# arkworks-rs/gemini

Measured on AMD Instinct MI355X. Metric: BLS12-381 G1 MSM throughput, higher is better.
Workload: dtype u32x12 Montgomery Fq (381-bit integer), u32x8 Fr; 1 GPU; 2^20 G1 MSM per GPU (BASELINE configs[1]: 2^20 G1 MSM on one MI355X); pairs_per_gpu=1048576

## Files before the change

gemini_amd/csrc/capi.hip:

```cpp
#include <cstring>
#include <vector>

#include "ctx.hpp"
#include "host_field.hpp"

namespace gm {

static thread_local char g_err[512] = "";
void set_error(const char* fmt, ...) {
  va_list ap;
  va_start(ap, fmt);
  vsnprintf(g_err, sizeof g_err, fmt, ap);
  va_end(ap);
}
int hip_fail(hipError_t e, const char* what, const char* file, int line) {
  set_error("HIP error %d (%s) in %s at %s:%d", (int)e, hipGetErrorString(e), what, file, line);
  return e == hipErrorOutOfMemory ? GM_ENOMEM : GM_EHIP;
}

MemStats& mem_stats() {
  static MemStats* m = new MemStats;
  return *m;
}
void MemStats::note_cached(ptrdiff_t delta) {
// ... 309 lines not shown
  if (const char* e = getenv("GM_POOL_MAX_GB")) C->pool.max_pooled = (size_t)strtoull(e, nullptr, 10) << 30;
  int prio_lo = 0, prio_hi = 0;
  GM_HIP(hipDeviceGetStreamPriorityRange(&prio_lo, &prio_hi));
  const bool prio = getenv("GM_STREAM_PRIO") && atoi(getenv("GM_STREAM_PRIO")) != 0;
  GM_HIP(hipStreamCreateWithPriority(&C->stream, hipStreamNonBlocking, prio ? prio_lo : 0));
  for (int k = 0; k < MSM_SMALL_LANES; k++) GM_HIP(hipStreamCreateWithPriority(&C->small_stream[k], hipStreamNonBlocking, prio ? prio_hi : 0));
  GM_HIP(hipStreamCreateWithPriority(&C->stream_b, hipStreamNonBlocking, prio ? prio_hi : 0));
  {
    const char* e = getenv("GM_CU_SPLIT");
    const int ncu = C->cu_count, per_xcd = ncu / 8;
    int T = e ? atoi(e) : (ncu == 256 ? per_xcd : 0);
    static const bool raw_env = getenv("GM_CU_SPLIT_RAW") != nullptr;
    if (!raw_env && per_xcd > 0) T = T / per_xcd * per_xcd;
    if (ncu % 8 == 0 && T > 0 && T < ncu) {
      const int words = (ncu + 31) / 32, xcds = T / per_xcd, stride = ncu / T;
      std::vector<uint32_t> m_tail((size_t)words, 0u), m_acc((size_t)words, 0u);
      int taken = 0;
      for (int i = 0; i < ncu; i++) {
        const bool tail = raw_env ? (taken < T && i % stride == 0) : (i % 8 < xcds);
        (tail ? m_tail : m_acc)[(size_t)i >> 5] |= 1u << (i & 31);
        taken += tail ? 1 : 0;
      }
      bool ok = true;
      for (int k = 0; k < 2 + MSM_SMALL_LANES && ok; k++) {
        ok = hipExtStreamCreateWithCUMask(&C->part_acc[k], (uint32_t)words, m_acc.data()) == hipSuccess &&
             hipExtStreamCreateWithCUMask(&C->part_tail[k], (uint32_t)words, m_tail.data()) == hipSuccess;
      }
      if (ok) {
        C->cu_split = T;
        static bool registered = false;
        if (!registered) {
          registered = true;
          atexit([] {
            Context* c = g_ctx;
            if (!c || !c->cu_split) return;
            c->cu_split = 0;
            for (int k = 0; k < 2 + MSM_SMALL_LANES; k++) {
              if (c->part_acc[k]) (void)hipStreamSynchronize(c->part_acc[k]), (void)hipStreamDestroy(c->part_acc[k]);
              if (c->part_tail[k]) (void)hipStreamSynchronize(c->part_tail[k]), (void)hipStreamDestroy(c->part_tail[k]);
              c->part_acc[k] = c->part_tail[k] = nullptr;
            }
          });
        }
      } else {
        (void)hipGetLastError();
      }
    }
  }
  GM_HIP(hipHostMalloc((void**)&C->host_small, 1 << 16, hipHostMallocDefault));
  GM_HIP(hipHostMalloc((void**)&C->sc_desc_host, SC_DESC_SLOTS * SC_DESC_SLOT, hipHostMallocDefault));
  GM_HIP(gm::raw_malloc(&C->sc_desc_dev, SC_DESC_SLOTS * SC_DESC_SLOT));
  for (auto& e : C->sc_desc_copied) GM_HIP(hipEventCreateWithFlags(&e, hipEventDisableTiming));
  if (const char* e = getenv("GM_ZERO_COPY")) C->zero_copy = atoi(e);
  g_ctx = C;
  return GM_OK;
}

void gm_shutdown(void) {
  std::lock_guard<std::mutex> lk(g_ctx_mu);
  if (!g_ctx) return;
  Context* C = g_ctx;
  (void)hipStreamSynchronize(C->stream);
  for (auto& kv : C->bases) {
    bases_free_tables(kv.second.get());
    if (kv.second->phi) (void)gm::raw_free(kv.second->phi);
    if (kv.second->d) (void)gm::raw_free(kv.second->d);
  }
  for (auto& kv : C->vecs)
    if (kv.second->d) (void)gm::raw_free(kv.second->d);
  for (auto& kv : C->msm_streams) msm_stream_destroy(C, kv.second.get());
  C->pool.release_all();
  for (auto& kv : C->provers) sc_destroy(kv.second.get());
  for (auto& kv : C->space_provers) sp_destroy(C, kv.second.get());
  for (auto& kv : C->herring_g1) hg1_destroy(C, kv.second.get());
  C->partial_bufs.release_all();
  for (auto& kv : C->indices)
    if (kv.second->d) (void)gm::raw_free(kv.second->d);
  for (auto& kv : C->matrices) {
    if (kv.second->rowptr) (void)gm::raw_free(kv.second->rowptr);
    if (kv.second->cols) (void)gm::raw_free(kv.second->cols);
    if (kv.second->vals) (void)gm::raw_free(kv.second->vals);
  }
  auto release_ws = [](MsmWorkspace& w) {
    for (DevBuf* b : {&w.scalars, &w.counts, &w.offsets, &w.cursor, &w.entries, &w.tmp_entries, &w.sortmeta, &w.buckets, &w.pk[0], &w.pk[1], &w.pp[0],
                      &w.pp[1], &w.rows, &w.cols, &w.planes, &w.misc, &w.lvl_cnt, &w.lvl_pos, &w.lvl_pts[0], &w.lvl_pts[1], &w.lvl_keys[0],
                      &w.lvl_keys[1], &w.lvl_prefix, &w.lvl_lane, &w.lvl_entries, &w.lvl_n})
      b->release();
    for (int k = 0; k < MSM_SLOTS; k++)
      if (w.host_planes[k]) (void)hipHostFree(w.host_planes[k]);
    if (w.have_done_ev) {
      for (int e = 0; e < MSM_SLOTS; e++) (void)hipEventDestroy(w.done_ev[e]);
    }
  };
  release_ws(C->msm);
  release_ws(C->msm_b);
  if (C->stream_b) (void)hipStreamDestroy(C->stream_b);
  for (int k = 0; k < MSM_SMALL_LANES; k++) {
    release_ws(C->msm_small[k]);
    if (C->small_stream[k]) (void)hipStreamDestroy(C->small_stream[k]);
  }
  for (int k = 0; k < 2 + MSM_SMALL_LANES; k++) {
    if (C->part_acc[k]) (void)hipStreamDestroy(C->part_acc[k]);
    if (C->part_tail[k]) (void)hipStreamDestroy(C->part_tail[k]);
  }
  C->cu_split = 0;
  if (C->host_small) (void)hipHostFree(C->host_small);
  if (C->sc_desc_host) (void)hipHostFree(C->sc_desc_host);
  if (C->sc_desc_dev) (void)gm::raw_free(C->sc_desc_dev);
  for (auto& e : C->sc_desc_copied)
    if (e) (void)hipEventDestroy(e);
  if (C->host_batch) (void)hipHostFree(C->host_batch);
  (void)hipStreamDestroy(C->stream);
  delete C;
  g_ctx = nullptr;
}

int gm_prof_enable(int on) {
  GM_CTX();
  C->prof.on = on != 0;
  C->prof.only_stage = on == 2 ? (int)PROF_ACC0 : -1;
  for (int s = 0; s < PROF_NSTAGES; s++) {
    C->prof.ms[s] = 0;
    C->prof.count[s] = 0;
    C->prof.pending[0][s] = C->prof.pending[1][s] = false;
  }
  C->prof.acc0_cycles = C->prof.acc0_ticks = 0;
  return GM_OK;
}
int gm_prof_read_clock(double* acc0_mhz) {
  GM_CTX();
  GM_CHECK(acc0_mhz != nullptr, GM_EINVAL, "prof_read_clock: null pointer");
  *acc0_mhz = C->prof.acc0_ticks > 0 ? C->prof.acc0_cycles / C->prof.acc0_ticks * 100.0 : 0.0;
  return GM_OK;
}
int gm_prof_read(double* ms_out, uint64_t* count_out, int n) {
  GM_CTX();
  GM_CHECK(n >= 0 && n <= PROF_NSTAGES, GM_EINVAL, "prof_read: n = %d, at most %d stages", n, (int)PROF_NSTAGES);
  for (int s = 0; s < n; s++) {
    if (ms_out) ms_out[s] = C->prof.ms[s];
    if (count_out) count_out[s] = C->prof.count[s];
  }
  return GM_OK;
}

int gm_set_msm_table_min(size_t n) {
  GM_CTX();
  C->msm_table_min = n;
  return GM_OK;
}

int gm_set_auto_tables(int on, size_t max_bytes) {
  GM_CTX();
  C->auto_tables = on != 0;
  C->auto_tables_max = max_bytes;
  return GM_OK;
}

int gm_pool_trim(void) {
  GM_CTX();
  C->pool.release_all();
  return GM_OK;
}

int gm_mem_stats(uint64_t out[12]) {
  GM_CTX();
  GM_CHECK(out != nullptr, GM_EINVAL, "gm_mem_stats: null output");
  size_t free_b = 0, total_b = 0;
// ... 1268 lines not shown
```

gemini_amd/csrc/ctx.hpp:

```cpp
#pragma once
#include <hip/hip_runtime.h>

#include <atomic>
#include <cstdarg>
#include <cstdint>
#include <cstdio>
#include <map>
#include <memory>
#include <mutex>
#include <string>
#include <unordered_map>
#include <vector>

#include "../../include/gemini_hip.h"

namespace gm {

void set_error(const char* fmt, ...);
int hip_fail(hipError_t e, const char* what, const char* file, int line);

#define GM_HIP(expr)                                                     \
  do {                                                                   \
    hipError_t _e = (expr);                                              \
    if (_e != hipSuccess) return ::gm::hip_fail(_e, #expr, __FILE__, __LINE__); \
// ... 68 lines not shown
  size_t round = 0, tot_rounds = 0;
  uint64_t pair_offset = 0;
  bool herring = false;
  uint8_t* partials = nullptr;
  uint64_t* host_partials = nullptr;
  unsigned pending_blocks = 0;
  bool on_host = false;
  std::vector<uint64_t> hf, hg;
  uint64_t host_msg[8];
  bool host_msg_pending = false;
  std::mutex mu;
};
constexpr size_t SC_HOST_TAIL = 256;
constexpr size_t SC_DESC_SLOT = (size_t)32 << 10;
constexpr unsigned SC_DESC_SLOTS = 8;

struct SpaceProver {
  uint8_t* f = nullptr;
  uint8_t* g = nullptr;
  size_t nf = 0, ng = 0, fcap = 0, gcap = 0;
  bool borrowed = false;
  std::vector<uint64_t> challenges, twisted;
  uint64_t twist[4];
  size_t round = 0, tot_rounds = 0;
  uint8_t* tables = nullptr;
  size_t tables_cap = 0;
  uint8_t *wf_lo = nullptr, *wf_hi = nullptr, *wg_lo = nullptr, *wg_hi = nullptr;
  uint8_t* partials = nullptr;
  uint64_t* host_partials = nullptr;
  std::mutex mu;
};

struct HerringG1 {
  uint8_t* f[2] = {nullptr, nullptr};
  uint8_t* g[2] = {nullptr, nullptr};
  size_t fcap[2] = {0, 0}, gcap[2] = {0, 0};
  int cur = 0;
  size_t nf = 0, ng = 0;
  uint64_t twist[4];
  size_t round = 0, tot_rounds = 0;
  uint8_t* tmp = nullptr;
  size_t tmpcap = 0;
  std::mutex mu;
};

struct MsmWorkspace;
struct MsmPending {
  MsmWorkspace* ws = nullptr;
  int slot = 0;
  bool empty = true;
  int Wb = 0, c = 0, m = 0;
  uint32_t nbits = 0, wf[3] = {0, 0, 0};
  size_t plane_off[3] = {0, 0, 0};
  size_t plane_count = 0;
  int multi_levels = 0;
  int multi_W = 0;
};
struct MsmStreamSlot {
  uint8_t *raw = nullptr, *packed = nullptr, *scalars = nullptr;
  size_t raw_cap = 0, packed_cap = 0, scalars_cap = 0;
  hipEvent_t copied;
  bool have_ev = false;
  bool inflight = false;
  MsmPending P;
};
struct MsmStream {
  std::mutex mu;
  size_t chunk = 0, stride = 96;
  int mont = 0;
  uint64_t bases_handle = 0;
  int64_t base0 = 0, next_base = 0, step = 1;
  MsmStreamSlot s[2];
  int cur = 0;
  size_t fill = 0, total = 0;
  hipStream_t copy = nullptr;
  uint64_t acc[18];
  bool acc_set = false;
};

constexpr int MSM_SLOTS = 4;
constexpr int MSM_SMALL_LANES = 6;
struct MsmWorkspace {
  DevBuf scalars, counts, offsets, cursor, entries, tmp_entries, sortmeta, buckets, pk[2], pp[2], rows, cols, planes, misc;
  DevBuf clk;
  DevBuf lvl_cnt, lvl_pos, lvl_pts[2], lvl_keys[2], lvl_prefix, lvl_lane, lvl_entries, lvl_n;
  uint64_t* host_planes[MSM_SLOTS] = {};
  size_t host_planes_cap[MSM_SLOTS] = {};
  hipEvent_t done_ev[MSM_SLOTS];
  hipEvent_t sort_ev, acc_ev;
  bool have_done_ev = false;
};

enum ProfStage { PROF_DIGITS = 0, PROF_SCAN, PROF_SCATTER, PROF_ACC0, PROF_MERGE, PROF_REDUCE, PROF_SC_ROUND, PROF_EXTFREQ, PROF_NSTAGES };
struct Profiler {
  bool on = false;
  int only_stage = -1;
  hipEvent_t ev[2][2 * PROF_NSTAGES];
  bool have_events = false;
  bool pending[2][PROF_NSTAGES] = {};
  double ms[PROF_NSTAGES] = {};
  uint64_t count[PROF_NSTAGES] = {};
  double acc0_cycles = 0, acc0_ticks = 0;
  void begin(int part, int stage, hipStream_t st);
  void end(int part, int stage, hipStream_t st);
  void begin(int stage, hipStream_t st) { begin(0, stage, st); }
  void end(int stage, hipStream_t st) { end(0, stage, st); }
  void collect();
};

struct DevPool {
  std::mutex mu;
  std::multimap<size_t, void*> free_list;
  size_t pooled_bytes = 0;
  size_t max_pooled = (size_t)96 << 30;
  int alloc(size_t bytes, void** p, size_t* cap);
  void free(void* p, size_t cap);
  void release_all();
};

struct PartialBufs {
  std::mutex mu;
  std::vector<std::pair<uint8_t*, uint64_t*>> free_pairs;
  int take(uint8_t** dev, uint64_t** host);
  void give(uint8_t* dev, uint64_t* host);
  void release_all();
};
constexpr size_t PARTIAL_BUF_BYTES = 512 * 2 * 32;

struct Context {
  int device = -1;
  PartialBufs partial_bufs;
  DevPool pool;
  Profiler prof;
  hipStream_t stream = nullptr;
  std::mutex mu;
  std::recursive_mutex msm_mu;
  std::recursive_mutex fr_mu;
  uint64_t next_handle = 1;
  std::unordered_map<uint64_t, std::unique_ptr<Bases>> bases;
  std::unordered_map<uint64_t, std::unique_ptr<FrVec>> vecs;
  std::unordered_map<uint64_t, std::unique_ptr<Sumcheck>> provers;
  std::unordered_map<uint64_t, std::unique_ptr<SparseMatrix>> matrices;
  std::unordered_map<uint64_t, std::unique_ptr<SpaceProver>> space_provers;
  std::unordered_map<uint64_t, std::unique_ptr<HerringG1>> herring_g1;
  std::unordered_map<uint64_t, std::unique_ptr<MsmStream>> msm_streams;
  std::unordered_map<uint64_t, std::unique_ptr<IdxVec>> indices;
  MsmWorkspace msm;
  MsmWorkspace msm_small[MSM_SMALL_LANES];
  hipStream_t small_stream[MSM_SMALL_LANES] = {};
  MsmWorkspace msm_b;
  hipStream_t stream_b = nullptr;
  int cu_split = 0;
  hipStream_t part_acc[2 + MSM_SMALL_LANES] = {};
  hipStream_t part_tail[2 + MSM_SMALL_LANES] = {};
  hipEvent_t start_ev;
  bool have_start_ev = false;
  DevBuf fr_scratch;
  uint64_t* host_small = nullptr;
  uint8_t* sc_desc_host = nullptr;
  uint8_t* sc_desc_dev = nullptr;
  hipEvent_t sc_desc_copied[SC_DESC_SLOTS] = {};
  unsigned sc_desc_next = 0;
  uint64_t* host_batch = nullptr;
  size_t host_batch_cap = 0;
  int msm_c_override = 0;
  int msm_glv = 0;
// ... 63 lines not shown
```

gemini_amd/csrc/msm.hip:

```cpp
#include <algorithm>
#include <atomic>
#include <chrono>
#include <condition_variable>
#include <cstdlib>
#include <cstring>
#include <functional>
#include <sched.h>
#include <cstdio>
#include <thread>
#include <vector>

#include "ctx.hpp"
#include "g1.cuh"
#include "host_field.hpp"

namespace gm {

constexpr uint32_t KEY_INV = 0xffffffffu;
constexpr int XYZZ_BYTES = 192;
constexpr int AFF_BYTES = 96;

struct DigitIter {
  uint32_t s[8];
  uint32_t carry;
// ... 830 lines not shown
      if (tab_stride) {
        const uint32_t lo = (uint32_t)e & 0x7fffffffu;
        idx = (long long)(lo >> ENTRY_W_SHIFT) * tab_stride + first + step * (long long)(lo & ((1u << ENTRY_W_SHIFT) - 1u));
      } else {
        idx = first + step * (long long)(e & 0x3fffffffull);
      }
      const uint8_t* src = (phi != nullptr && ((e >> ENTRY_HALF_SHIFT) & 1ull)) ? phi : bases;
      return reinterpret_cast<const gm_u4v*>(src + (size_t)idx * AFF_BYTES);
    };
    uint64_t e = entry_at(start);
    const gm_u4v* bp = base_of(e);
    gm_u4v x0 = bp[0], x1 = bp[1], x2 = bp[2], y0 = bp[3], y1 = bp[4], y2 = bp[5];
    for (uint64_t i = start; i < end; i++) {
      uint64_t en = 0;
      gm_u4v n0 = x0, n1 = x1, n2 = x2, n3 = y0, n4 = y1, n5 = y2;
      if (i + 1 < end) {
        en = entry_at(i + 1);
        const gm_u4v* np = base_of(en);
        asm volatile(
            "global_load_dwordx4 %0, %6, off\n\t"
            "global_load_dwordx4 %1, %6, off offset:16\n\t"
            "global_load_dwordx4 %2, %6, off offset:32\n\t"
            "global_load_dwordx4 %3, %6, off offset:48\n\t"
            "global_load_dwordx4 %4, %6, off offset:64\n\t"
            "global_load_dwordx4 %5, %6, off offset:80"
            : "=&v"(n0), "=&v"(n1), "=&v"(n2), "=&v"(n3), "=&v"(n4), "=&v"(n5)
            : "v"(np));
      }
      const uint32_t key = (uint32_t)(e >> 32);
      if (key != cur) {
        if (cur != KEY_INV) {
          if (first_run) {
            head_key = cur;
            acc30_store(pp + (size_t)(2 * (size_t)t) * XYZZ30_BYTES, acc);
            first_run = false;
          } else {
            acc30_store(buckets + (size_t)cur * XYZZ30_BYTES, acc);
          }
        }
        cur = key;
        acc30_set_identity(acc);
      }
      const uint32_t nz = x0.x | x0.y | x0.z | x0.w | x1.x | x1.y | x1.z | x1.w | x2.x | x2.y | x2.z | x2.w | y0.x | y0.y | y0.z | y0.w |
                          y1.x | y1.y | y1.z | y1.w | y2.x | y2.y | y2.z | y2.w;
      if (nz != 0) {
        const uint32_t neg = (uint32_t)(e >> 31) & 1u;
        (void)g1_madd30_asm(acc, x0, x1, x2, y0, y1, y2, neg);
      }
      asm volatile("s_waitcnt vmcnt(0)" : "+v"(n0), "+v"(n1), "+v"(n2), "+v"(n3), "+v"(n4), "+v"(n5));
      e = en;
      x0 = n0; x1 = n1; x2 = n2; y0 = n3; y1 = n4; y2 = n5;
    }
    if (first_run) {
      head_key = cur;
      acc30_store(pp + (size_t)(2 * (size_t)t) * XYZZ30_BYTES, acc);
    } else {
      tail_key = cur;
      acc30_store(pp + (size_t)(2 * (size_t)t + 1) * XYZZ30_BYTES, acc);
    }
  }
  pk[2 * (size_t)t] = head_key;
  pk[2 * (size_t)t + 1] = tail_key;
  if (t == 0 && clk != nullptr) {
    clk[0] = (unsigned long long)(clock64() - clk_c0);
    clk[1] = (unsigned long long)(wall_clock64() - clk_w0);
  }
}

#ifdef GM_EXPERIMENTS
#include "msm_levels.inc"
#endif

__global__ __launch_bounds__(64) void k_merge(const uint32_t* __restrict__ keys_in, const uint8_t* __restrict__ pts_in,
                                              uint32_t E, uint32_t* __restrict__ keys_out,
                                              uint8_t* __restrict__ pts_out, uint8_t* __restrict__ buckets,
                                              int final_level) {
  __shared__ __attribute__((aligned(16))) uint8_t lds[128 * XYZZ30_BYTES];
  const int lane = threadIdx.x;
  const uint32_t wave = blockIdx.x;
  const uint32_t s0 = wave * 128u + 2u * lane;
  uint32_t hk = s0 < E ? keys_in[s0] : KEY_INV;
  uint32_t tk = s0 + 1 < E ? keys_in[s0 + 1] : KEY_INV;
  uint32_t hs = 2 * lane, ts = 2 * lane + 1;
  auto copy_rec = [](void* dst, const void* src) {
    const gm_u4v* s = reinterpret_cast<const gm_u4v*>(src);
    gm_u4v* d = reinterpret_cast<gm_u4v*>(dst);
#pragma unroll
    for (int i = 0; i < 13; i++) d[i] = s[i];
  };
  auto add_slots = [&](uint32_t dst_slot, uint32_t src_slot, Acc30& a) {
    Acc30 o;
    acc30_load(a, lds + dst_slot * XYZZ30_BYTES);
    acc30_load(o, lds + src_slot * XYZZ30_BYTES);
    acc30_add(a, o);
  };
  if (hk != KEY_INV) copy_rec(lds + hs * XYZZ30_BYTES, pts_in + (size_t)s0 * XYZZ30_BYTES);
  if (tk != KEY_INV) copy_rec(lds + ts * XYZZ30_BYTES, pts_in + ((size_t)s0 + 1) * XYZZ30_BYTES);
  if (hk == KEY_INV && tk != KEY_INV) {
    hk = tk;
    hs = ts;
    tk = KEY_INV;
  }
  __syncthreads();
  if (hk != KEY_INV && hk == tk) {
    Acc30 a;
    add_slots(hs, ts, a);
    acc30_store(lds + hs * XYZZ30_BYTES, a);
    tk = KEY_INV;
  }
  __syncthreads();

  {
    const uint32_t nhk = __shfl_down(hk, 1), nhs = __shfl_down(hs, 1), ntk = __shfl_down(tk, 1);
    const uint32_t ptk = __shfl_up(tk, 1);
    const bool give = lane < 63 && tk != KEY_INV && ntk != KEY_INV && nhk == tk;
    const bool taken = lane > 0 && tk != KEY_INV && ptk != KEY_INV && ptk == hk;
    if (__any(give)) {
      if (give) {
        Acc30 a;
        add_slots(ts, nhs, a);
        acc30_store(buckets + (size_t)tk * XYZZ30_BYTES, a);
      }
    }
    __syncthreads();
    if (taken) {
      hk = tk; hs = ts; tk = KEY_INV;
    }
    if (give) {
      if (taken) { hk = KEY_INV; } else { tk = KEY_INV; }
    }
  }

  for (int d = 1; d < 64; d <<= 1) {
    const uint32_t bhk = __shfl_down(hk, d), bhs = __shfl_down(hs, d);
    const uint32_t btk = __shfl_down(tk, d), bts = __shfl_down(ts, d);
    const bool act = (lane & (2 * d - 1)) == 0;
    bool do_add = false;
    uint32_t add_dst = 0, add_src = 0;
    uint32_t f1k = KEY_INV, f1s = 0, f2k = KEY_INV, f2s = 0;
    if (act && bhk != KEY_INV) {
      if (hk == KEY_INV) {
        hk = bhk; hs = bhs; tk = btk; ts = bts;
      } else {
        const bool a_two = tk != KEY_INV, b_two = btk != KEY_INV;
        const uint32_t alk = a_two ? tk : hk, als = a_two ? ts : hs;
        if (alk == bhk) {
          do_add = true; add_dst = als; add_src = bhs;
          if (b_two) {
            if (a_two) { f1k = alk; f1s = als; }
            tk = btk; ts = bts;
          }
        } else {
          if (a_two) { f1k = tk; f1s = ts; }
          if (b_two) { f2k = bhk; f2s = bhs; tk = btk; ts = bts; }
          else { tk = bhk; ts = bhs; }
        }
      }
    }
    if (__any(do_add)) {
      if (do_add) {
        Acc30 a;
        add_slots(add_dst, add_src, a);
        acc30_store(lds + add_dst * XYZZ30_BYTES, a);
      }
    }
    if (f1k != KEY_INV) copy_rec(buckets + (size_t)f1k * XYZZ30_BYTES, lds + f1s * XYZZ30_BYTES);
    if (f2k != KEY_INV) copy_rec(buckets + (size_t)f2k * XYZZ30_BYTES, lds + f2s * XYZZ30_BYTES);
    __syncthreads();
  }
  if (lane == 0) {
    if (final_level) {
      if (hk != KEY_INV) copy_rec(buckets + (size_t)hk * XYZZ30_BYTES, lds + hs * XYZZ30_BYTES);
      if (tk != KEY_INV) copy_rec(buckets + (size_t)tk * XYZZ30_BYTES, lds + ts * XYZZ30_BYTES);
    } else {
      keys_out[2 * (size_t)wave] = hk;
      keys_out[2 * (size_t)wave + 1] = tk;
      if (hk != KEY_INV) copy_rec(pts_out + (size_t)(2 * (size_t)wave) * XYZZ30_BYTES, lds + hs * XYZZ30_BYTES);
      if (tk != KEY_INV) copy_rec(pts_out + (size_t)(2 * (size_t)wave + 1) * XYZZ30_BYTES, lds + ts * XYZZ30_BYTES);
    }
  }
}

enum { GS_STRIDED = 0, GS_PLANE = 1 };
struct GroupSumArgs {
  const uint8_t* in;
  uint8_t* out;
  int mode;
  uint32_t n_out;
  uint32_t per_win;
  uint32_t win_stride;
  uint32_t n_lo, s_hi, s_lo, s_e, len;
  uint32_t nb;
  uint32_t lpo_shift;
  int out_canonical;
  const uint32_t* in_cnt;
};
struct GroupSumJobs {
  GroupSumArgs j[3];
  uint32_t blk_end[3];
  const uint32_t* err_src;
  uint32_t* err_dst;
  const unsigned long long* clk_src;
};

__global__ __launch_bounds__(256) void k_group_sum(GroupSumJobs J) {
  if (J.err_dst && blockIdx.x == 0 && threadIdx.x == 0) {
    *J.err_dst = *J.err_src;
    if (J.clk_src) {
      unsigned long long* d = reinterpret_cast<unsigned long long*>(J.err_dst + 2);
      d[0] = J.clk_src[0];
      d[1] = J.clk_src[1];
    }
  }
  const int job = blockIdx.x < J.blk_end[0] ? 0 : (blockIdx.x < J.blk_end[1] ? 1 : 2);
  const GroupSumArgs& a = J.j[job];
  const uint32_t blk0 = job == 0 ? 0u : J.blk_end[job - 1];
  const uint8_t* __restrict__ in = a.in;
  uint8_t* __restrict__ out = a.out;
  const uint32_t gt = (blockIdx.x - blk0) * blockDim.x + threadIdx.x;
  const uint32_t lpo = 1u << a.lpo_shift;
  const uint32_t o = gt >> a.lpo_shift, q = gt & (lpo - 1u);
  Acc30 acc;
  acc30_zero(acc);
  const uint32_t* __restrict__ in_cnt = a.in_cnt;
  auto filled = [&](size_t slot) { return in_cnt == nullptr || in_cnt[slot] != 0u; };
  auto add_rec = [&](size_t slot) {
    if (!filled(slot)) return;
    Acc30 v;
    acc30_load(v, in + slot * XYZZ30_BYTES);
    acc30_add(acc, v);
  };
  auto load_first = [&](size_t slot) {
    if (filled(slot)) acc30_load(acc, in + slot * XYZZ30_BYTES);
  };
  if (o < a.n_out) {
    const uint32_t w = o / a.per_win, r = o % a.per_win;
    const size_t base = (size_t)w * a.win_stride;
    if (a.mode == GS_STRIDED) {
      const size_t b0 = base + (size_t)(r / a.n_lo) * a.s_hi + (size_t)(r % a.n_lo) * a.s_lo;
      if (q < a.len) load_first(b0 + (size_t)q * a.s_e);
      for (uint32_t e = q + lpo; e < a.len; e += lpo) add_rec(b0 + (size_t)e * a.s_e);
    } else {
      const uint32_t nb = a.nb;
      if (r == nb) {
        const uint32_t cnt0 = nb ? (1u << (nb - 1)) : 1u;
        if (q < cnt0) load_first(base + 2u * q);
        for (uint32_t e = q + lpo; e < cnt0; e += lpo) add_rec(base + 2u * e);
      } else {
        const uint32_t half = nb ? (1u << (nb - 1)) : 0u;
        auto slot_of = [&](uint32_t e) { return ((e >> r) << (r + 1)) | (1u << r) | (e & ((1u << r) - 1u)); };
        if (q < half) load_first(base + slot_of(q));
        for (uint32_t e = q + lpo; e < half; e += lpo) add_rec(base + slot_of(e));
      }
    }
  }
#pragma unroll 1
  for (int m = (int)(lpo >> 1); m >= 1; m >>= 1) {
    Acc30 other;
    acc30_shfl_xor(other, acc, m);
    acc30_add(acc, other);
  }
  if (o < a.n_out && q == 0) {
    if (a.out_canonical) g1_store_xyzz(out + (size_t)o * XYZZ_BYTES, acc30_to_canonical(acc));
// ... 125 lines not shown
}

__global__ __launch_bounds__(256) void k_fixed_base_mul(const uint32_t* __restrict__ scalars, int mont, size_t n,
                                                        const uint8_t* __restrict__ table_aff, uint8_t* __restrict__ out_xyzz) {
  size_t i = (size_t)blockIdx.x * blockDim.x + threadIdx.x;
  if (i >= n) return;
  Fr s = fp_load<FrParams>(scalars + 8 * i);
  if (mont) s = fp_from_mont<FrParams>(s);
  G1Xyzz acc = G1Xyzz::identity();
  for (int w = 0; w < 32; w++) {
    uint32_t dgt = (s.l[w >> 2] >> (8 * (w & 3))) & 255u;
    if (dgt) {
      G1Affine p = g1_load_affine(table_aff + ((size_t)w * 256 + dgt) * AFF_BYTES);
      xyzz_madd(acc, p);
    }
  }
  g1_store_xyzz(out_xyzz + i * XYZZ_BYTES, acc);
}

__global__ __launch_bounds__(256) void k_g1_split_fold(const uint8_t* __restrict__ in, size_t n, const uint32_t* __restrict__ s8,
                                                       uint8_t* __restrict__ out) {
  const size_t m = (n + 1) / 2;
  size_t i = (size_t)blockIdx.x * blockDim.x + threadIdx.x;
  if (i >= m) return;
  G1Affine lo = g1_load_affine(in + (2 * i) * AFF_BYTES);
  G1Xyzz acc = G1Xyzz::identity();
  if (2 * i + 1 < n) {
    G1Affine hi = g1_load_affine(in + (2 * i + 1) * AFF_BYTES);
    for (int bit = 254; bit >= 0; bit--) {
      acc = xyzz_dbl(acc);
      if ((s8[bit >> 5] >> (bit & 31)) & 1u) xyzz_madd(acc, hi);
    }
  }
  xyzz_madd(acc, lo);
  G1Affine a;
  if (acc.is_identity()) {
    a.x = fqe_zero();
    a.y = fqe_zero();
  } else {
    FqE t = fq_mul(acc.zz, acc.zzz);
    FqE ti = fq_inv(t);
    a.x = fq_mul(acc.x, fq_mul(ti, acc.zzz));
    a.y = fq_mul(acc.y, fq_mul(ti, acc.zz));
  }
  g1_store_affine(out + i * AFF_BYTES, a);
}

__global__ __launch_bounds__(256) void k_table_next(const uint8_t* __restrict__ prev, uint8_t* __restrict__ next_xyzz, size_t n, int c) {
  size_t i = (size_t)blockIdx.x * blockDim.x + threadIdx.x;
  if (i >= n) return;
  G1Affine p = g1_load_affine(prev + i * AFF_BYTES);
  G1Xyzz acc = G1Xyzz::from_affine(p);
  for (int k = 0; k < c; k++) acc = xyzz_dbl(acc);
  g1_store_xyzz(next_xyzz + i * XYZZ_BYTES, acc);
}

static int ceil_log2_sz(size_t n) {
  int b = 0;
  size_t v = n > 1 ? n - 1 : 0;
  while (v) {
    b++;
    v >>= 1;
  }
  return b;
}

static int choose_window(size_t n) {
  int lg = ceil_log2_sz(n);
  static const size_t c20_min = getenv("GM_MSM_C20_MIN") ? (size_t)strtoull(getenv("GM_MSM_C20_MIN"), nullptr, 10) : ((size_t)7 << 21);
  if (n >= c20_min) return 20;
  if (lg >= 23) return 19;
  static const int c_medium = getenv("GM_MSM_C_MEDIUM") ? atoi(getenv("GM_MSM_C_MEDIUM")) : 0;
  if (c_medium && lg >= 14 && lg <= 17) return c_medium;
  if (lg >= 14) return 16;
  if (lg >= 11) return 8;
  if (lg >= 8) return lg - 4;
  if (lg >= 5) return lg + 1;
  return 4;
}

size_t msm_workspace_held(const MsmWorkspace& ws) {
  size_t b = 0;
  for (const DevBuf* d : {&ws.scalars, &ws.counts, &ws.offsets, &ws.cursor, &ws.entries, &ws.tmp_entries, &ws.sortmeta, &ws.buckets, &ws.pk[0], &ws.pk[1],
                          &ws.pp[0], &ws.pp[1], &ws.rows, &ws.cols, &ws.planes, &ws.misc, &ws.clk})
    b += d->cap;
  return b;
}
size_t msm_workspace_bound(Context* C, const Bases* bases, size_t n) {
  if (n == 0) return 0;
  n = std::min<size_t>(n, (size_t)1 << 26);
  int c = C->msm_c_override ? C->msm_c_override : choose_window(n);
  bool table = false;
  if (bases && !C->msm_c_override && n < ((size_t)1 << ENTRY_W_SHIFT)) {
    if (bases->table && n >= std::max(C->msm_table_min, bases->tab_min)) {
      c = bases->tab_c;
      table = true;
    } else {
      for (const Bases::TableSet& ts : bases->extra)
        if (n >= ts.min_n && n < ts.max_n && n <= ts.n) {
          c = ts.c;
          table = true;
          break;
        }
    }
  }
  const size_t W = (size_t)(256 + c - 1) / (size_t)c;
  const size_t N = n * W, nbuckets = (table ? 1 : W) << (c - 1);
  auto grow = [](size_t b) { return b + b / 8 + 256; };
  const size_t lanes0 = N >= ((size_t)1 << 24) ? 262144 : 131072;
  const size_t L = std::min<size_t>(256, std::max<size_t>(4, (N + lanes0 - 1) / lanes0)) + 1;
  const size_t E1 = 2 * ((N / L + 256 + 255) / 256 * 256), E2 = 2 * ((E1 + 127) / 128);
  size_t b = 2 * grow(N * 8);
  b += grow(nbuckets * XYZZ30_BYTES) + 4 * grow((nbuckets + 8192) * 4);
  b += grow(E1 * 4) + grow(E1 * XYZZ30_BYTES) + grow(E2 * 4) + grow(E2 * XYZZ30_BYTES);
  b += (size_t)W * ((size_t)3 << 14) * XYZZ30_BYTES + ((size_t)16 << 20);
  return b;
}

constexpr size_t MSM_SMALL_N = (size_t)1 << 17;
constexpr size_t MSM_SPLIT_MIN_N = (size_t)1 << 17;
static int msm_run_one(Context* C, const Bases* bases, int64_t first, int64_t step, const void* d_scalars, int mont, size_t n,
                       bool normalize, uint64_t out_jac[18]);
static int msm_run_batch_at(Context* C, const Bases* bases, int64_t first, int64_t step, const size_t* pair_offsets, const void* const* d_scalars,
                            int mont, const size_t* ns, size_t k, bool normalize, uint64_t* out_jac, const int64_t* firsts = nullptr);

struct MsmStreams {
  hipStream_t sort, acc, tail;
};
struct MsmMulti {
  bool block = false;
  int levels = 0;
  const void* scalars[MULTI_MAX_LEVELS];
  size_t n[MULTI_MAX_LEVELS];
  int64_t start[MULTI_MAX_LEVELS];
};
constexpr size_t MSM_MULTI_MAX_N = (size_t)1 << 13;
constexpr size_t MSM_MULTI_BLOCK_MAX_N = (size_t)1 << 20;
static int msm_enqueue(Context* C, MsmWorkspace& ws, MsmStreams sts, const Bases* bases, int64_t first, int64_t step, const void* d_scalars,
                       int mont, size_t n, int slot, MsmPending* P, int part = 0, int nparts = 1, const MsmMulti* multi = nullptr);
static int msm_finish_parts(Context* C, const MsmPending* parts, int nparts, bool normalize, uint64_t out_jac[18], bool use_pool = true,
                            uint64_t* const* multi_out = nullptr);
static void horner_pool_prewake();
static void horner_pool_run(int n, const std::function<void(int)>& fn);
static int msm_finish(Context* C, const MsmPending& P, bool normalize, uint64_t out_jac[18], bool use_pool = true) {
  return msm_finish_parts(C, &P, 1, normalize, out_jac, use_pool);
}

int msm_run(Context* C, const Bases* bases, int64_t first, int64_t step, const void* d_scalars, int mont, size_t n,
            bool normalize, uint64_t out_jac[18]) {
  const size_t CH = (size_t)1 << 26;
  if (n <= CH) return msm_run_one(C, bases, first, step, d_scalars, mont, n, normalize, out_jac);
  gmh::G1 acc = gmh::G1::identity();
  for (size_t off = 0; off < n; off += CH) {
    const size_t m = n - off < CH ? n - off : CH;
    uint64_t part[18];
    int rc = msm_run_one(C, bases, first + step * (int64_t)off, step, reinterpret_cast<const uint8_t*>(d_scalars) + off * 32, mont, m, false, part);
    if (rc) return rc;
    acc = acc.add(gmh::G1::from_limbs(part));
  }
  if (normalize) acc = acc.normalized();
  acc.to_limbs(out_jac);
  return GM_OK;
}

static int msm_run_one(Context* C, const Bases* bases, int64_t first, int64_t step, const void* d_scalars, int mont, size_t n,
                       bool normalize, uint64_t out_jac[18]) {
  GM_MSM_LOCK(C);
  const bool tables = bases->table != nullptr && !C->msm_c_override && n >= std::max(C->msm_table_min, bases->tab_min) &&
                      n < ((size_t)1 << ENTRY_W_SHIFT);
  const bool split = GM_GLV(1) && C->msm_split && n >= MSM_SPLIT_MIN_N && !tables && C->msm_affine_levels == 0 && C->stream_b && C->small_stream[0];
  if (!split) {
    MsmPending P;
    int rc = msm_enqueue(C, C->msm, MsmStreams{C->stream, C->stream, C->stream}, bases, first, step, d_scalars, mont, n, 0, &P);
    if (rc) return rc;
    return msm_finish(C, P, normalize, out_jac);
  }
  if (!C->have_start_ev) {
    GM_HIP(hipEventCreateWithFlags(&C->start_ev, hipEventDisableTiming));
    C->have_start_ev = true;
  }
  GM_HIP(hipEventRecord(C->start_ev, C->stream));
  GM_HIP(hipStreamWaitEvent(C->small_stream[0], C->start_ev, 0));
  MsmPending P[2];
  const MsmStreams sts{C->small_stream[0], C->stream, C->stream_b};
  const MsmStreams sts_lo{C->small_stream[0], C->stream, C->small_stream[1]};
  int rc = msm_enqueue(C, C->msm, sts, bases, first, step, d_scalars, mont, n, 0, &P[1], 1, 2);
  if (!rc) rc = msm_enqueue(C, C->msm_b, sts_lo, bases, first, step, d_scalars, mont, n, 0, &P[0], 0, 2);
  if (rc) {
    (void)hipStreamSynchronize(C->small_stream[0]);
    (void)hipStreamSynchronize(C->stream);
    (void)hipStreamSynchronize(C->stream_b);
    (void)hipStreamSynchronize(C->small_stream[1]);
    return rc;
  }
  return msm_finish_parts(C, P, 2, normalize, out_jac);
}

// ... 324 lines not shown
      return tn <= ((size_t)1 << ENTRY_W_SHIFT);
    };
    if (bases->table != nullptr && bases->tab_c <= 20 && covers(bases->n)) {
      tab_ptr = bases->table;
      tab_c_sel = bases->tab_c;
      tab_n = bases->n;
    } else {
      for (const Bases::TableSet& ts : bases->extra)
        if (ts.c <= 20 && ts.c >= 18 && covers(ts.n)) {
          tab_ptr = ts.t;
          tab_c_sel = ts.c;
          tab_n = ts.n;
          break;
        }
    }
  }
  if (!multi && !C->msm_c_override && n < ((size_t)1 << ENTRY_W_SHIFT)) {
    if (bases->table != nullptr && n >= tab_min) {
      tab_ptr = bases->table;
      tab_c_sel = bases->tab_c;
      tab_n = bases->n;
    } else if (C->msm_table_min <= ((size_t)1 << 17) || n >= C->msm_table_min) {
      const int64_t last = first + step * (int64_t)(n - 1);
      for (const Bases::TableSet& ts : bases->extra)
        if (n >= ts.min_n && n < ts.max_n && first >= 0 && last >= 0 && (size_t)first < ts.n && (size_t)last < ts.n) {
          tab_ptr = ts.t;
          tab_c_sel = ts.c;
          tab_n = ts.n;
          break;
        }
    }
  }
  const bool use_table = tab_ptr != nullptr;
  const bool multi_block = multi && multi->block;
  static const int fuse_c_env = getenv("GM_MSM_FUSE_C") ? atoi(getenv("GM_MSM_FUSE_C")) : 16;
  const int c = multi ? (multi_block ? (use_table ? tab_c_sel : fuse_c_env) : 8) : (use_table ? tab_c_sel : (C->msm_c_override ? C->msm_c_override : choose_window(n)));
  GM_CHECK(c >= 2 && c <= 22, GM_EINVAL, "msm: window width %d out of range [2, 22]", c);
  static const bool sort_atomic_env0 = getenv("GM_MSM_SORT") && !strcmp(getenv("GM_MSM_SORT"), "atomic");
  static const int acc0_waves = getenv("GM_ACC0_WAVES") ? atoi(getenv("GM_ACC0_WAVES")) : 2;
  const size_t bucket_bytes = XYZZ30_BYTES;
  const bool use_glv = GM_GLV(1) && !multi && bases->phi != nullptr && !use_table && C->msm_affine_levels == 0 && !sort_atomic_env0 && n <= ((size_t)1 << 26);
  const int W = ((use_glv ? 128 : 256) + c - 1) / c;
  GM_CHECK(nparts == 1 || !use_table, GM_EINVAL, "msm: the fixed-base table path is not split into window groups");
  const int w_lo = part * W / nparts, Wg = (part + 1) * W / nparts - w_lo;
  const uint32_t B = 1u << (c - 1);
  const int Wb = multi ? multi->levels * (use_table ? 1 : W) : (use_table ? 1 : Wg);
  const size_t nbuckets = (size_t)Wb * B;
  const uint8_t* d_bases = use_table ? tab_ptr : bases->d;
  const long long tab_stride = use_table ? (long long)tab_n : 0;
  const uint64_t Nall = (uint64_t)n * (uint64_t)W * (use_glv ? 2u : 1u);
  const uint64_t N = (uint64_t)n * (uint64_t)(use_table ? W : Wg) * (use_glv ? 2u : 1u);
  GM_CHECK(Nall < (1ull << 32), GM_EINVAL, "msm: n*W = %llu entries exceed 2^32; chunk the stream", (unsigned long long)Nall);

  int levels = C->msm_affine_levels;
  if (levels < 0) {
    levels = 0;
    if (N >= ((uint64_t)1 << 22))
      for (uint64_t avg = N / nbuckets; avg >= 8 && levels < 6; avg >>= 1) levels++;
  }
  GM_CHECK(levels <= 8, GM_EINVAL, "msm: %d affine levels (max 8)", levels);
  uint64_t Nacc = N;
  for (int l = 0; l < levels; l++) Nacc = Nacc / 2 + 2 * nbuckets + 2;

  static const int L_env = getenv("GM_MSM_L") ? atoi(getenv("GM_MSM_L")) : 0;
  const uint64_t Nacc_all = nparts > 1 ? Nall : Nacc;
  const uint64_t lanes0 = Nacc_all >= ((uint64_t)1 << 24) ? 262144 : 131072;
  static const uint64_t L_cap = getenv("GM_MSM_LCAP") ? (uint64_t)atoi(getenv("GM_MSM_LCAP")) : 256;
  uint32_t L = (uint32_t)std::min<uint64_t>(L_cap, std::max<uint64_t>(4, (Nacc_all + lanes0 - 1) / lanes0));
  if (L_env > 0) L = (uint32_t)L_env;
  L = (L + 1u) & ~1u;
  const uint64_t T0 = (Nacc + L - 1) / L;
  const uint64_t T0pad = (T0 + 255) / 256 * 256;
  const uint64_t E1 = 2 * T0pad;

  int rc;
  const size_t counts_words = (nbuckets + 2 + SORT_GMAX + 1 + 63) / 64 * 64;
  if ((rc = ws.counts.ensure(counts_words * 4))) return rc;
  if ((rc = ws.offsets.ensure((nbuckets + 1) * 4))) return rc;
  if ((rc = ws.cursor.ensure((nbuckets + 1) * 4))) return rc;
  if ((rc = ws.misc.ensure((nbuckets / SCAN_PER_BLOCK + 2) * 4))) return rc;
  if ((rc = ws.entries.ensure(N * 8))) return rc;
  if ((rc = ws.buckets.ensure(nbuckets * bucket_bytes))) return rc;
  if ((rc = ws.pk[0].ensure(E1 * 4))) return rc;
  if ((rc = ws.pp[0].ensure(E1 * bucket_bytes))) return rc;
  const uint64_t E2 = 2 * ((E1 + 127) / 128);
  if ((rc = ws.pk[1].ensure(E2 * 4))) return rc;
  if ((rc = ws.pp[1].ensure(E2 * bucket_bytes))) return rc;

  const uint32_t* sc = reinterpret_cast<const uint32_t*>(d_scalars);
  GM_HIP(hipMemsetAsync(ws.counts.p, 0, counts_words * 4, st));
  uint32_t* d_err = ws.counts.as<uint32_t>() + nbuckets + 1;
  const bool bucket_counts_valid = levels == 0;
  if (!bucket_counts_valid) GM_HIP(hipMemsetAsync(ws.buckets.p, 0, nbuckets * bucket_bytes, st));
  const uint32_t dblocks = (uint32_t)((n + 255) / 256);
  Profiler& pf = C->prof;
  auto run_scan = [&]() {
    const uint32_t nb = (uint32_t)((nbuckets + SCAN_PER_BLOCK - 1) / SCAN_PER_BLOCK);
    hipLaunchKernelGGL(k_scan_block_sums, dim3(nb), dim3(256), 0, st, ws.counts.as<uint32_t>(), (uint32_t)nbuckets,
                       ws.misc.as<uint32_t>());
    hipLaunchKernelGGL(k_scan_top, dim3(1), dim3(1024), 0, st, ws.misc.as<uint32_t>(), nb,
                       ws.offsets.as<uint32_t>() + nbuckets);
    hipLaunchKernelGGL(k_scan_apply, dim3(nb), dim3(256), 0, st, ws.counts.as<uint32_t>(), (uint32_t)nbuckets,
                       ws.misc.as<uint32_t>(), ws.offsets.as<uint32_t>(), ws.cursor.as<uint32_t>());
  };
  static const bool sort_atomic_env = getenv("GM_MSM_SORT") && !strcmp(getenv("GM_MSM_SORT"), "atomic");
  static const bool sort_flat_env = !(getenv("GM_MSM_SORT") && !strcmp(getenv("GM_MSM_SORT"), "blocks"));
  const bool sort_atomic = sort_atomic_env && !use_table && nparts == 1 && !multi_block;
  const bool sort_flat = sort_flat_env && !sort_atomic && !use_table && nparts == 1 && !multi_block && N <= ((uint64_t)1 << 21) && nbuckets <= ((size_t)1 << 18);
  LevelGeom lg{};
  if (multi_block) {
    lg.levels = multi->levels;
    lg.step = (int)step;
    uint32_t at = 0;
    for (int l = 0; l < multi->levels; l++) {
      lg.start[l] = at;
      lg.scal[l] = reinterpret_cast<const uint32_t*>(multi->scalars[l]);
      lg.base0[l] = (long long)multi->start[l];
      at += (uint32_t)multi->n[l];
    }
    lg.start[multi->levels] = at;
  }
  if (multi && !multi_block) {
    MultiGeom mg{};
    mg.c = c;
    mg.W = W;
    mg.levels = multi->levels;
    mg.step = (int)step;
    mg.B = B;
    for (int j = 0; j + 1 < W; j++) {
      const int b = c * j + c - 1;
      if (b < 256) mg.K[b >> 5] |= 1u << (b & 31);
    }
    uint32_t at = 0;
    for (int l = 0; l < multi->levels; l++) {
      mg.start[l] = at;
      mg.scal[l] = reinterpret_cast<const uint32_t*>(multi->scalars[l]);
      mg.base0[l] = (long long)multi->start[l];
      at += (uint32_t)multi->n[l];
    }
    mg.start[multi->levels] = at;
    GM_CHECK(N <= ((uint64_t)1 << 21) && nbuckets <= ((size_t)1 << 18), GM_EINVAL, "msm: fused calls too large for the flat sort (%llu entries, %zu buckets)",
             (unsigned long long)N, nbuckets);
    const dim3 grid((uint32_t)((n + 255) / 256), (uint32_t)W);
    pf.begin(part, PROF_DIGITS, st);
    hipLaunchKernelGGL(k_digits_multi<false>, grid, dim3(256), 0, st, mg, mont, ws.counts.as<uint32_t>(), (uint64_t*)nullptr, d_err);
    hipLaunchKernelGGL(k_scan_small, dim3(1), dim3(1024), 0, st, ws.counts.as<uint32_t>(), (uint32_t)nbuckets, ws.offsets.as<uint32_t>(),
                       ws.cursor.as<uint32_t>());
    pf.end(part, PROF_DIGITS, st);
    pf.begin(part, PROF_SCATTER, st);
    hipLaunchKernelGGL(k_digits_multi<true>, grid, dim3(256), 0, st, mg, mont, ws.cursor.as<uint32_t>(), ws.entries.as<uint64_t>(), d_err);
    pf.end(part, PROF_SCATTER, st);
  } else if (sort_flat) {
    FlatGeom fg{};
    fg.c = c;
    fg.W = W;
    fg.glv = use_glv ? 1 : 0;
    fg.B = B;
    for (int j = 0; j + 1 < W; j++) {
      const int b = c * j + c - 1;
      if (b < 256) fg.K[b >> 5] |= 1u << (b & 31);
    }
    const dim3 grid((uint32_t)((n + 255) / 256), (uint32_t)(W * (use_glv ? 2 : 1)));
    pf.begin(part, PROF_DIGITS, st);
    hipLaunchKernelGGL(k_digits_flat<false>, grid, dim3(256), 0, st, sc, (uint32_t)n, mont, fg, ws.counts.as<uint32_t>(), (uint64_t*)nullptr, d_err);
    hipLaunchKernelGGL(k_scan_small, dim3(1), dim3(1024), 0, st, ws.counts.as<uint32_t>(), (uint32_t)nbuckets, ws.offsets.as<uint32_t>(),
                       ws.cursor.as<uint32_t>());
// ... 29 lines not shown
    GM_CHECK(sg.G <= SORT_GMAX, GM_EINVAL, "msm: %u coarse sort bins exceed %u (window %d too wide for this sort)", sg.G, SORT_GMAX, c);
    if ((rc = ws.tmp_entries.ensure(N * 8))) return rc;
    if ((rc = ws.sortmeta.ensure((size_t)(3 * (sg.G + 1)) * 4))) return rc;
    uint32_t* gcount = ws.counts.as<uint32_t>() + nbuckets + 2;
    uint32_t* goff = ws.sortmeta.as<uint32_t>();
    uint32_t* gcursor = goff + (sg.G + 1);
    uint32_t* blkoff = gcursor + (sg.G + 1);
    const uint32_t b1 = (uint32_t)((n + SORT_TS - 1) / SORT_TS);
    const uint32_t b2 = (uint32_t)(N / SORT_CH + sg.G + 1);
    pf.begin(part, PROF_DIGITS, st);
    hipLaunchKernelGGL(k_sort1<false>, dim3(b1), dim3(256), 0, st, sc, (uint32_t)n, mont, sg, lg, gcount, (uint64_t*)nullptr, d_err);
    hipLaunchKernelGGL(k_sort1_scan, dim3(1), dim3(1024), 0, st, gcount, sg.G, goff, gcursor, blkoff);
    const size_t stage1_lds = (size_t)SORT_TS * sg.Wg * (use_glv ? 2 : 1) * 8 + (size_t)3 * sg.G * 4 + 1024 * 4;
    static const bool sort1_staged_env = !(getenv("GM_MSM_SORT1") && !strcmp(getenv("GM_MSM_SORT1"), "direct"));
    if (sort1_staged_env && sg.Wg * (use_glv ? 2 : 1) <= SORT1_STAGE_WMAX && stage1_lds <= 160 * 1024) {
      static bool attr_set = false;
      if (!attr_set) {
        GM_HIP(hipFuncSetAttribute(reinterpret_cast<const void*>(k_sort1_staged), hipFuncAttributeMaxDynamicSharedMemorySize, 160 * 1024));
        attr_set = true;
      }
      hipLaunchKernelGGL(k_sort1_staged, dim3(b1), dim3(1024), stage1_lds, st, sc, (uint32_t)n, mont, sg, lg, gcursor, ws.tmp_entries.as<uint64_t>());
    } else {
      hipLaunchKernelGGL(k_sort1<true>, dim3(b1), dim3(256), 0, st, sc, (uint32_t)n, mont, sg, lg, gcursor, ws.tmp_entries.as<uint64_t>(), d_err);
    }
    pf.end(part, PROF_DIGITS, st);
    pf.begin(part, PROF_SCATTER, st);
    hipLaunchKernelGGL(k_sort2<false>, dim3(b2), dim3(256), 0, st, ws.tmp_entries.as<uint64_t>(), goff, blkoff, sg,
                       ws.counts.as<uint32_t>(), (uint64_t*)nullptr);
    run_scan();
    static const bool sort_staged = !(getenv("GM_MSM_SORT2") && !strcmp(getenv("GM_MSM_SORT2"), "direct"));
    if (sort_staged && (1u << sg.FB) <= SORT_STAGE_FMAX)
      hipLaunchKernelGGL(k_sort2_staged, dim3(b2), dim3(1024), 0, st, ws.tmp_entries.as<uint64_t>(), goff, blkoff, sg,
                         ws.cursor.as<uint32_t>(), ws.entries.as<uint64_t>());
    else
      hipLaunchKernelGGL(k_sort2<true>, dim3(b2), dim3(256), 0, st, ws.tmp_entries.as<uint64_t>(), goff, blkoff, sg,
                         ws.cursor.as<uint32_t>(), ws.entries.as<uint64_t>());
    pf.end(part, PROF_SCATTER, st);
  }
  const uint64_t* acc_entries = ws.entries.as<uint64_t>();
  const uint32_t* acc_total = ws.offsets.as<uint32_t>() + nbuckets;
  const uint8_t* acc_bases = d_bases;
  long long acc_first = (long long)first, acc_step = multi ? 1ll : (long long)step, acc_tab = tab_stride;
#ifdef GM_EXPERIMENTS
#define GM_MSM_LEVELS_HOST 1
#include "msm_levels.inc"
#undef GM_MSM_LEVELS_HOST
#else
  GM_CHECK(levels == 0, GM_EINVAL, "msm: affine tree levels are an experiment of round 2; rebuild with -DGM_EXPERIMENTS (DESIGN.md section 8)");
#endif
  if (!ws.have_done_ev) {
    for (int e = 0; e < MSM_SLOTS; e++) GM_HIP(hipEventCreateWithFlags(&ws.done_ev[e], hipEventDisableTiming));
    GM_HIP(hipEventCreateWithFlags(&ws.sort_ev, hipEventDisableTiming));
    GM_HIP(hipEventCreateWithFlags(&ws.acc_ev, hipEventDisableTiming));
    ws.have_done_ev = true;
  }
  if (sts.acc != st) {
    GM_HIP(hipEventRecord(ws.sort_ev, st));
    GM_HIP(hipStreamWaitEvent(sts.acc, ws.sort_ev, 0));
  }
  st = sts.acc;
  pf.begin(part, PROF_ACC0, st);
  static const size_t acc0_lds_pad = getenv("GM_ACC0_LDS_PAD") ? (size_t)strtoull(getenv("GM_ACC0_LDS_PAD"), nullptr, 10) : 0;
  if ((rc = ws.clk.ensure(16))) return rc;
  unsigned long long* acc_clk = ws.clk.as<unsigned long long>();
  static const int acc0_pf_env = getenv("GM_ACC0_PREFETCH") ? atoi(getenv("GM_ACC0_PREFETCH")) : -1;
  const bool acc0_pf = acc0_pf_env >= 0 ? acc0_pf_env != 0 : use_table;
  if (acc0_pf)
    hipLaunchKernelGGL(k_acc0_pf<2>, dim3((uint32_t)(T0pad / 256)), dim3(256), 0, st, acc_entries, acc_total, acc_bases, acc_first, acc_step,
                       acc_tab, L, ws.pk[0].as<uint32_t>(), ws.pp[0].as<uint8_t>(), ws.buckets.as<uint8_t>(), use_glv ? bases->phi : (const uint8_t*)nullptr, acc_clk);
  else if (acc0_waves == 2)
    hipLaunchKernelGGL(k_acc0<2>, dim3((uint32_t)(T0pad / 256)), dim3(256), acc0_lds_pad, st, acc_entries, acc_total, acc_bases, acc_first, acc_step,
                       acc_tab, L, ws.pk[0].as<uint32_t>(), ws.pp[0].as<uint8_t>(), ws.buckets.as<uint8_t>(), use_glv ? bases->phi : (const uint8_t*)nullptr, acc_clk);
  else
    hipLaunchKernelGGL(k_acc0<3>, dim3((uint32_t)(T0pad / 256)), dim3(256), 0, st, acc_entries, acc_total, acc_bases, acc_first, acc_step,
                       acc_tab, L, ws.pk[0].as<uint32_t>(), ws.pp[0].as<uint8_t>(), ws.buckets.as<uint8_t>(), use_glv ? bases->phi : (const uint8_t*)nullptr, acc_clk);
  pf.end(part, PROF_ACC0, st);
  if (sts.tail != st) {
    GM_HIP(hipEventRecord(ws.acc_ev, st));
    GM_HIP(hipStreamWaitEvent(sts.tail, ws.acc_ev, 0));
  }
  st = sts.tail;
  pf.begin(part, PROF_MERGE, st);
  {
    uint64_t E = E1;
    int src = 0;
    for (;;) {
      uint32_t waves = (uint32_t)((E + 127) / 128);
      int final_level = waves == 1;
      hipLaunchKernelGGL(k_merge, dim3(waves), dim3(64), 0, st, ws.pk[src].as<uint32_t>(), ws.pp[src].as<uint8_t>(),
                         (uint32_t)E, ws.pk[src ^ 1].as<uint32_t>(), ws.pp[src ^ 1].as<uint8_t>(),
                         ws.buckets.as<uint8_t>(), final_level);
      if (final_level) break;
      E = 2ull * waves;
      src ^= 1;
    }
  }

  pf.end(part, PROF_MERGE, st);
  pf.begin(part, PROF_REDUCE, st);
  const uint32_t nbits = (uint32_t)(c - 1);
  uint32_t wf[3] = {0, 0, 0};
  int m;
  static const int fields_env = getenv("GM_MSM_FIELDS") ? atoi(getenv("GM_MSM_FIELDS")) : 0;
  if (nbits <= 7) {
    m = 1;
    wf[0] = nbits;
  } else if (nbits <= 14 || (fields_env == 2 && nbits <= 16)) {
    m = 2;
    wf[0] = nbits / 2;
    wf[1] = nbits - wf[0];
  } else {
    m = 3;
    static const bool odd_low = !(getenv("GM_MSM_ODD_BIT") && !strcmp(getenv("GM_MSM_ODD_BIT"), "high"));
    wf[0] = odd_low ? (nbits + 2) / 3 : nbits / 3;
    wf[1] = (nbits - wf[0]) / 2;
    wf[2] = nbits - wf[0] - wf[1];
  }
  static const int lpo_env = getenv("GM_MSM_LPO_LOG") ? atoi(getenv("GM_MSM_LPO_LOG")) : 0;
  const int lpo_target_log = lpo_env ? lpo_env : (nbuckets >= ((size_t)1 << 21) ? 18 : 17);
  uint32_t lpo_jobs = 1;
  auto lpo_for = [&](uint32_t len, uint32_t n_out) {
    uint32_t s = 0;
    while (s < 5 && (1u << s) < len && ((uint64_t)n_out << s) * lpo_jobs < (1ull << lpo_target_log)) s++;
    return s;
  };
  const uint8_t* bucket_in = ws.buckets.as<uint8_t>();
  const uint32_t* bucket_cnt = bucket_counts_valid ? ws.counts.as<uint32_t>() : nullptr;
  auto strided = [&](const uint8_t* in, uint8_t* out, uint32_t win_in, uint32_t n_hi, uint32_t n_lo, uint32_t s_hi, uint32_t s_lo,
                     uint32_t s_e, uint32_t len) {
    GroupSumArgs g{};
    g.in = in; g.out = out; g.mode = GS_STRIDED; g.in_cnt = in == bucket_in ? bucket_cnt : nullptr;
    g.per_win = n_hi * n_lo; g.n_out = (uint32_t)Wb * g.per_win; g.win_stride = win_in;
    g.n_lo = n_lo; g.s_hi = s_hi; g.s_lo = s_lo; g.s_e = s_e; g.len = len; g.lpo_shift = lpo_for(len, g.n_out);
    return g;
  };
  auto plane = [&](const uint8_t* in, uint8_t* out, uint32_t nb) {
    GroupSumArgs g{};
    g.in = in; g.out = out; g.mode = GS_PLANE; g.out_canonical = 1;
    g.in_cnt = in == bucket_in ? bucket_cnt : nullptr;
    g.per_win = nb + 1; g.n_out = (uint32_t)Wb * g.per_win; g.win_stride = 1u << nb; g.nb = nb;
    g.lpo_shift = lpo_for(nb ? (1u << (nb - 1)) : 1u, g.n_out);
    return g;
  };
  uint8_t* planes = nullptr;
  size_t plane_count = 0;
  auto launch = [&](std::initializer_list<GroupSumArgs> jobs, bool last = false) {
    GroupSumJobs J{};
    if (last) {
      J.err_src = d_err;
      J.err_dst = reinterpret_cast<uint32_t*>(planes + plane_count * XYZZ_BYTES);
      J.clk_src = ws.clk.as<unsigned long long>();
    }
    uint32_t tot = 0;
    int k = 0;
    for (const GroupSumArgs& g : jobs) {
      J.j[k] = g;
      tot += (uint32_t)((((uint64_t)g.n_out << g.lpo_shift) + 255) / 256);
      J.blk_end[k] = tot;
      k++;
    }
    for (; k < 3; k++) J.blk_end[k] = tot;
    hipLaunchKernelGGL(k_group_sum, dim3(tot), dim3(256), 0, st, J);
  };
  size_t plane_off[3];
  for (int k = 0; k < m; k++) {
    plane_off[k] = plane_count;
    plane_count += (size_t)Wb * (wf[k] + 1);
  }
  const size_t plane_bytes = plane_count * XYZZ_BYTES + 24;
  if (ws.host_planes_cap[slot] < plane_bytes) {
    if (ws.host_planes[slot]) (void)hipHostFree(ws.host_planes[slot]);
    ws.host_planes[slot] = nullptr;
    ws.host_planes_cap[slot] = 0;
    GM_HIP(hipHostMalloc((void**)&ws.host_planes[slot], plane_bytes, hipHostMallocDefault));
    ws.host_planes_cap[slot] = plane_bytes;
  }
  const bool zc = (C->zero_copy & 2) != 0;
// ... 740 lines not shown
```

Baseline: 348.7 Mscalar/s.

## Resolve accumulator-chunk boundaries in a pre-pass and skip empty merge waves

Adds a k_boundary kernel that looks at adjacent thread outputs from acc0 (head/tail key pairs). It either adds the two records that share a bucket or writes whole buckets straight into the bucket array, then marks those keys invalid in a separate key buffer. k_merge gains an early exit when no lane in the wave holds two valid keys, so the first merge level can skip most waves. The cost is an extra kernel launch, an extra key buffer of E1 words, and more reasoning needed about bucket ownership correctness.

Result: no change. 349.4 Mscalar/s (median of 4 runs) (+0.2%).

```diff
diff --git a/gemini_amd/csrc/capi.hip b/gemini_amd/csrc/capi.hip
--- a/gemini_amd/csrc/capi.hip
+++ b/gemini_amd/csrc/capi.hip
@@ -415,7 +415,7 @@
     if (kv.second->vals) (void)gm::raw_free(kv.second->vals);
   }
   auto release_ws = [](MsmWorkspace& w) {
-    for (DevBuf* b : {&w.scalars, &w.counts, &w.offsets, &w.cursor, &w.entries, &w.tmp_entries, &w.sortmeta, &w.buckets, &w.pk[0], &w.pk[1], &w.pp[0],
+    for (DevBuf* b : {&w.scalars, &w.counts, &w.offsets, &w.cursor, &w.entries, &w.tmp_entries, &w.sortmeta, &w.buckets, &w.pk[0], &w.pk[1], &w.pkb, &w.pp[0],
                       &w.pp[1], &w.rows, &w.cols, &w.planes, &w.misc, &w.lvl_cnt, &w.lvl_pos, &w.lvl_pts[0], &w.lvl_pts[1], &w.lvl_keys[0],
                       &w.lvl_keys[1], &w.lvl_prefix, &w.lvl_lane, &w.lvl_entries, &w.lvl_n})
       b->release();
diff --git a/gemini_amd/csrc/ctx.hpp b/gemini_amd/csrc/ctx.hpp
--- a/gemini_amd/csrc/ctx.hpp
+++ b/gemini_amd/csrc/ctx.hpp
@@ -174,6 +174,7 @@
 constexpr int MSM_SMALL_LANES = 6;
 struct MsmWorkspace {
   DevBuf scalars, counts, offsets, cursor, entries, tmp_entries, sortmeta, buckets, pk[2], pp[2], rows, cols, planes, misc;
+  DevBuf pkb;
   DevBuf clk;
   DevBuf lvl_cnt, lvl_pos, lvl_pts[2], lvl_keys[2], lvl_prefix, lvl_lane, lvl_entries, lvl_n;
   uint64_t* host_planes[MSM_SLOTS] = {};
diff --git a/gemini_amd/csrc/msm.hip b/gemini_amd/csrc/msm.hip
--- a/gemini_amd/csrc/msm.hip
+++ b/gemini_amd/csrc/msm.hip
@@ -936,6 +936,13 @@
   uint32_t hk = s0 < E ? keys_in[s0] : KEY_INV;
   uint32_t tk = s0 + 1 < E ? keys_in[s0 + 1] : KEY_INV;
   uint32_t hs = 2 * lane, ts = 2 * lane + 1;
+  if (!__any((hk & tk) != KEY_INV)) {
+    if (!final_level && lane == 0) {
+      keys_out[2 * (size_t)wave] = KEY_INV;
+      keys_out[2 * (size_t)wave + 1] = KEY_INV;
+    }
+    return;
+  }
   auto copy_rec = [](void* dst, const void* src) {
     const gm_u4v* s = reinterpret_cast<const gm_u4v*>(src);
     gm_u4v* d = reinterpret_cast<gm_u4v*>(dst);
@@ -1033,6 +1040,45 @@
       if (tk != KEY_INV) copy_rec(pts_out + (size_t)(2 * (size_t)wave + 1) * XYZZ30_BYTES, lds + ts * XYZZ30_BYTES);
     }
   }
+}
+
+__global__ __launch_bounds__(256) void k_boundary(const uint32_t* __restrict__ keys_in, const uint8_t* __restrict__ pts, uint32_t T,
+                                                  uint32_t* __restrict__ keys_out, uint8_t* __restrict__ buckets) {
+  const uint32_t b = blockIdx.x * blockDim.x + threadIdx.x;
+  if (b > T) return;
+  uint32_t phk = KEY_INV, ptk = KEY_INV, uhk = KEY_INV, utk = KEY_INV;
+  if (b > 0) {
+    const uint2 k = reinterpret_cast<const uint2*>(keys_in)[b - 1];
+    phk = k.x; ptk = k.y;
+  }
+  if (b < T) {
+    const uint2 k = reinterpret_cast<const uint2*>(keys_in)[b];
+    uhk = k.x; utk = k.y;
+  }
+  const bool p_two = ptk != KEY_INV, u_two = utk != KEY_INV;
+  const uint32_t p_last = p_two ? ptk : phk;
+  const bool join = p_two && u_two && uhk == ptk;
+  const bool tail_whole = p_two && uhk != ptk;
+  const bool head_whole = u_two && p_last != uhk;
+  const uint8_t* head_rec = pts + (size_t)2 * b * XYZZ30_BYTES;
+  const uint8_t* tail_rec = head_rec - XYZZ30_BYTES;
+  auto copy_rec = [](void* dst, const void* src) {
+    const gm_u4v* s = reinterpret_cast<const gm_u4v*>(src);
+    gm_u4v* d = reinterpret_cast<gm_u4v*>(dst);
+#pragma unroll
+    for (int i = 0; i < 13; i++) d[i] = s[i];
+  };
+  if (join) {
+    Acc30 a, o;
+    acc30_load(a, tail_rec);
+    acc30_load(o, head_rec);
+    acc30_add(a, o);
+    acc30_store(buckets + (size_t)ptk * XYZZ30_BYTES, a);
+  }
+  if (tail_whole) copy_rec(buckets + (size_t)ptk * XYZZ30_BYTES, tail_rec);
+  if (head_whole) copy_rec(buckets + (size_t)uhk * XYZZ30_BYTES, head_rec);
+  if (b > 0) keys_out[2 * (size_t)b - 1] = (join || tail_whole) ? KEY_INV : ptk;
+  if (b < T) keys_out[2 * (size_t)b] = (join || head_whole) ? KEY_INV : uhk;
 }
 
 enum { GS_STRIDED = 0, GS_PLANE = 1 };
@@ -1324,7 +1370,7 @@
 size_t msm_workspace_held(const MsmWorkspace& ws) {
   size_t b = 0;
   for (const DevBuf* d : {&ws.scalars, &ws.counts, &ws.offsets, &ws.cursor, &ws.entries, &ws.tmp_entries, &ws.sortmeta, &ws.buckets, &ws.pk[0], &ws.pk[1],
-                          &ws.pp[0], &ws.pp[1], &ws.rows, &ws.cols, &ws.planes, &ws.misc, &ws.clk})
+                          &ws.pkb, &ws.pp[0], &ws.pp[1], &ws.rows, &ws.cols, &ws.planes, &ws.misc, &ws.clk})
     b += d->cap;
   return b;
 }
@@ -1354,7 +1400,7 @@
   const size_t E1 = 2 * ((N / L + 256 + 255) / 256 * 256), E2 = 2 * ((E1 + 127) / 128);
   size_t b = 2 * grow(N * 8);
   b += grow(nbuckets * XYZZ30_BYTES) + 4 * grow((nbuckets + 8192) * 4);
-  b += grow(E1 * 4) + grow(E1 * XYZZ30_BYTES) + grow(E2 * 4) + grow(E2 * XYZZ30_BYTES);
+  b += 2 * grow(E1 * 4) + grow(E1 * XYZZ30_BYTES) + grow(E2 * 4) + grow(E2 * XYZZ30_BYTES);
   b += (size_t)W * ((size_t)3 << 14) * XYZZ30_BYTES + ((size_t)16 << 20);
   return b;
 }
@@ -1845,6 +1891,7 @@
   if ((rc = ws.entries.ensure(N * 8))) return rc;
   if ((rc = ws.buckets.ensure(nbuckets * bucket_bytes))) return rc;
   if ((rc = ws.pk[0].ensure(E1 * 4))) return rc;
+  if ((rc = ws.pkb.ensure(E1 * 4))) return rc;
   if ((rc = ws.pp[0].ensure(E1 * bucket_bytes))) return rc;
   const uint64_t E2 = 2 * ((E1 + 127) / 128);
   if ((rc = ws.pk[1].ensure(E2 * 4))) return rc;
@@ -2040,17 +2087,21 @@
   st = sts.tail;
   pf.begin(part, PROF_MERGE, st);
   {
+    hipLaunchKernelGGL(k_boundary, dim3((uint32_t)(T0pad / 256) + 1u), dim3(256), 0, st, ws.pk[0].as<uint32_t>(), ws.pp[0].as<uint8_t>(),
+                       (uint32_t)T0pad, ws.pkb.as<uint32_t>(), ws.buckets.as<uint8_t>());
     uint64_t E = E1;
     int src = 0;
+    const uint32_t* keys_in = ws.pkb.as<uint32_t>();
     for (;;) {
       uint32_t waves = (uint32_t)((E + 127) / 128);
       int final_level = waves == 1;
-      hipLaunchKernelGGL(k_merge, dim3(waves), dim3(64), 0, st, ws.pk[src].as<uint32_t>(), ws.pp[src].as<uint8_t>(),
+      hipLaunchKernelGGL(k_merge, dim3(waves), dim3(64), 0, st, keys_in, ws.pp[src].as<uint8_t>(),
                          (uint32_t)E, ws.pk[src ^ 1].as<uint32_t>(), ws.pp[src ^ 1].as<uint8_t>(),
                          ws.buckets.as<uint8_t>(), final_level);
       if (final_level) break;
       E = 2ull * waves;
       src ^= 1;
+      keys_in = ws.pk[src].as<uint32_t>();
     }
   }
 
```
